# waleedbinkhalid74/cnn-gp

Measured on AMD Instinct MI355X. Metric: kernel entries/s (N×M pairs) + full-Kxx build+solve wall-clock, MNIST 28×28, higher is better.
Workload: dtype f64; 1 GPU; mnist_paper_convnet_gp Kxx 4096x4096, tiles 1024; n=4096, tile=1024, parallelism=tiles-dp1

## Files before the change

### cnn-gp_amd/csrc/net_walk.inc

```
    for (long long u = advance(); u < end; u = advance()) {
        if (tid == 0) grab = atomicAdd(ctr, 1ull);
        Pairs pr;
        pr.tab = pair_tab;
        pr.u0 = u;
        pr.red = red_part;
        if constexpr (NP == 2) {
            const int q = __builtin_amdgcn_readfirstlane(tid >> 7);
            unsigned iq = 0, jq = 0;
            bool vq = false, wq = false, any = false;
#pragma unroll
            for (int s = 0; s < UN; ++s) {
                unsigned is = 0, js = 0;
                const bool vs = u + s < end && unit_pair(p, u + s, is, js);
                const bool ws = vs && !(p.same && js <= is);
                any |= ws;
                if (s == q) {
                    iq = is;
                    jq = js;
                    vq = vs;
                    wq = ws;
                }
            }
            if (!any) {
                if (p.final_stage && p.same && (tid & (kNT - 1)) == 0 && vq && jq == iq)
                    p.out[(long long)iq * p.ldo + iq] = p.kdiag[iq];
                continue;
            }
            Pairs ph;
            ph.tab = pair_tab;
            ph.u0 = u + q;
            ph.red = red_part + q * (kNT / 64);
            ph.i = __builtin_amdgcn_readfirstlane(vq ? iq : 0u);
            ph.j = __builtin_amdgcn_readfirstlane(vq ? jq : 0u);
            T* lh = lds + q * p.lds_elems;
            const int ht = tid & (kNT - 1);
            if constexpr (PID < 0) {
                for (int k = 0; k < p.nops; ++k) {
                    const cgp_net_op op = load_op(ops_c(p.ops) + k);
                    net_op<T, EX, DU, 1>(lh, op, p, ph, ht);
                    lds_barrier();
                }
            } else {
                prog_ops<T, DU, 1, PID, 0, CGP_WALK_LEAN>(lh, p, ph, ht, prog_recs, hx);
            }
            if (p.final_stage && ht == 0 && vq) {
                if (wq) {
                    const T v = lh[p.final_slot];
                    p.out[(long long)ph.i * p.ldo + ph.j] = v;
                    if (p.same) p.out[(long long)ph.j * p.ldo + ph.i] = v;
                } else if (ph.j == ph.i) {
                    p.out[(long long)ph.i * p.ldo + ph.i] = p.kdiag[ph.i];
                }
            }
        } else {
            if constexpr (NP == 1) {
                if (!unit_pair(p, u, pr.i, pr.j)) continue;
                pr.i = __builtin_amdgcn_readfirstlane(pr.i);
                pr.j = __builtin_amdgcn_readfirstlane(pr.j);
                if (p.same && pr.j <= pr.i) {
                    if (p.final_stage && pr.j == pr.i && tid == 0)
                        p.out[(long long)pr.i * p.ldo + pr.i] = p.kdiag[pr.i];
                    continue;
                }
            } else {
                if (tid < NP) {
                    unsigned iq = 0, jq = 0;
                    unit_pair(p, u + tid, iq, jq);
                    pair_tab[tid] = iq < p.n1 ? iq : p.n1 - 1;
                    pair_tab[kMaxNP + tid] = jq < p.n2 ? jq : p.n2 - 1;
                }
                pr.i = pr.j = 0;
                lds_barrier();
            }
            if constexpr (PID < 0) {
                for (int k = 0; k < p.nops; ++k) {
                    const cgp_net_op op = load_op(ops_c(p.ops) + k);
                    net_op<T, EX, DU, NP>(lds, op, p, pr, tid);
                    lds_barrier();
                }
            } else {
                prog_ops<T, DU, NP, PID, 0, CGP_WALK_LEAN>(lds, p, pr, tid, prog_recs, hx);
            }
            if (p.final_stage) {
                if constexpr (NP == 1) {
                    if (tid == 0) {
                        const T v = lds[p.final_slot];
                        p.out[(long long)pr.i * p.ldo + pr.j] = v;
                        if (p.same) p.out[(long long)pr.j * p.ldo + pr.i] = v;
                    }
                } else if (tid < NP) {
                    unsigned iq, jq;
                    if (u + tid < end && unit_pair(p, u + tid, iq, jq)) {
                        if (!p.same || jq > iq) {
                            const T v = lds[tid * p.lds_elems + p.final_slot];
                            p.out[(long long)iq * p.ldo + jq] = v;
                            if (p.same) p.out[(long long)jq * p.ldo + iq] = v;
                        } else if (jq == iq) {
                            p.out[(long long)iq * p.ldo + iq] = p.kdiag[iq];
                        }
                    }
                }
            }
        }
        lds_barrier();
    }
```

### cnn-gp_amd/csrc/netfuse.hip

```cpp

#include "cgp_common.h"


#include <map>
#include <mutex>
#include <utility>
#include <algorithm>
#include <climits>

using namespace cgp;

namespace {

constexpr int kNT = 128;
constexpr int kSplit = 2;
template <int NP>
constexpr int kNTof = NP == 2 ? kSplit * kNT : kNT;
template <int NP>
constexpr int kUnitsOf = NP == 2 ? kSplit : NP;
constexpr int kSTL = 3;
constexpr int kST = 1 << kSTL;
constexpr int kEw = 4;

constexpr int pick_r(int lines, int len, int taps, int s, int epi, int nt) {
// ... 1046 lines not shown

#define CGP_NET_RES_CASE(h, w)                                                        \
    case res_index(h, w):                                                             \
        if constexpr (CGP_NET_FITS(h, w)) net_elem<T, EX, DU, KIND, h, w, NP>(lds, op, p, pr); \
        break;

template <typename T, bool EX, bool DU, int KIND, int NP>
__device__ __forceinline__ void net_elem_dispatch(T* __restrict__ lds, const cgp_net_op& op,
                                                  const NetP<T>& p, const Pairs& pr) {
    if constexpr (KIND == CGP_NET_RELU || (KIND == CGP_NET_LINEAR && NP > 1)) {
        switch (op.code) {
            CGP_NET_RESOLUTIONS(CGP_NET_RES_CASE)
        default:
            if constexpr (NP == 1) net_elem<T, EX, DU, KIND, 0, 0, 1>(lds, op, p, pr);
            break;
        }
    } else if constexpr (NP == 1) {
        net_elem<T, EX, DU, KIND, 0, 0, 1>(lds, op, p, pr);
    }
}

template <typename T, bool EX, bool DU, int NP>
__device__ __forceinline__ void net_op(T* __restrict__ lds, const cgp_net_op& op,
                                       const NetP<T>& p, const Pairs& pr, int tid) {
    if (op.zero_halo) {
#pragma unroll
        for (int q = 0; q < NP; ++q) {
            const int qa = NP == 1 ? 0 : q * p.lds_elems;
            zero_halos<T, kNT>(lds + qa, op.dst, op.zero_halo & 0xffff, op.h, op.w,
                                     op.ws_out, tid);
            zero_halos<T, kNT>(lds + qa, op.dst2, (unsigned)op.zero_halo >> 16, op.h, op.w,
                       op.ws_out, tid);
        }
    }
    switch (op.kind) {
    case CGP_NET_CONV:
        switch (op.code & CGP_NET_CODE_GEOMETRY) {
            CGP_NET_GEOMETRIES(CGP_NET_CASE)
        default:
            break;
        }
        break;
    case CGP_NET_RELU:
        net_elem_dispatch<T, EX, DU, CGP_NET_RELU, NP>(lds, op, p, pr);
        break;
    case CGP_NET_MOMENTS:
        net_elem_dispatch<T, EX, DU, CGP_NET_MOMENTS, NP>(lds, op, p, pr);
        break;
    case CGP_NET_LINEAR:
        net_elem_dispatch<T, EX, DU, CGP_NET_LINEAR, NP>(lds, op, p, pr);
        break;
    case CGP_NET_LOAD:
        net_move<T, CGP_NET_LOAD, NP>(lds, op, p, pr);
        break;
    case CGP_NET_STORE:
        net_move<T, CGP_NET_STORE, NP>(lds, op, p, pr);
        break;
    default:
        break;
    }
}

#ifndef CGP_NET_PRESCALE
#define CGP_NET_PRESCALE 1
#endif
constexpr bool kNetPrescale = CGP_NET_PRESCALE != 0;
struct ProgOp {
    int kind, code, src, dst, add, ws_in, ws_out, relu, h, w, dst2, zero_halo;
};
struct ProgInfo {
    int first, nops, pairs, dual, lds_elems, sizes;
};
#include "net_programs.h"
constexpr int kNumProgs = sizeof(kProgs) / sizeof(kProgs[0]);

struct ProgRec {
    double weight, bias;
    const void* var_x;
    const void* var_y;
    const void* var2_x;
    const void* var2_y;
};
template <int PID>
constexpr int kRecsOf = PID >= 0 ? kProgs[PID < 0 ? 0 : PID].nops : 1;

template <int PID, int K>
__device__ __forceinline__ cgp_net_op prog_op(const ProgRec* recs) {
    constexpr ProgOp o = kProgOps[kProgs[PID].first + K];
    const ProgRec& rt = recs[K];
    cgp_net_op op;
    op.kind = o.kind;
    op.code = o.code;
    op.src = o.src;
    op.dst = o.dst;
    op.add = o.add;
    op.ws_in = o.ws_in;
    op.ws_out = o.ws_out;
    op.relu = o.relu;
    op.h = o.h;
    op.w = o.w;
    op.div_m = 0;
    op.div_s = 0;
    op.dst2 = o.dst2;
    op.zero_halo = o.zero_halo;
    op.weight = rt.weight;
    op.bias = rt.bias;
    op.var_x = rt.var_x;
    op.var_y = rt.var_y;
    op.var2_x = rt.var2_x;
    op.var2_y = rt.var2_y;
    return op;
}
template <int PID, int K, int NP>
struct ProgGeo {
    static constexpr ProgOp o = kProgOps[kProgs[PID].first + K];
    static constexpr GeoRow g = kGeoTable[o.code & CGP_NET_CODE_GEOMETRY];
    using G = NG<g.h, g.w, g.ho, g.wo, g.taps, g.s, g.off, NP>;
};
__host__ __device__ inline bool lean_rec_ok(double w, double b) {
    return w >= 0.0 && w <= 0x1p60 && b >= 0x1p-60 && b <= 0x1p60;
}
constexpr int kMaxProgOps = 24;
struct LeanOp {
    bool nocap = false, half = false, dbl = false;
};
struct ProgLean {
    LeanOp op[kMaxProgOps] = {};
    unsigned dbl_mask = 0;
    int capfree = 0, addfree = 0;
    int nend = 0, end_lo[4] = {}, end_hi[4] = {};
    bool bad = false;
};
struct LeanFact {
    int lo = 0, hi = 0;
    bool nonneg = false, halved = false;
};
constexpr bool lean_overlap(int lo, int hi, int lo2, int hi2) { return lo < hi2 && lo2 < hi; }
constexpr bool op_is_sum(const ProgOp& o) {
    return o.kind == CGP_NET_CONV && (o.code & CGP_NET_CODE_SUM) != 0;
}
constexpr int op_src_hi(const ProgOp& o) {
    if (o.kind == CGP_NET_CONV) return o.src + kGeoTable[o.code & CGP_NET_CODE_GEOMETRY].h * o.ws_in;
    if (o.kind == CGP_NET_RELU || o.kind == CGP_NET_LINEAR || o.kind == CGP_NET_STORE)
        return o.src + o.h * o.ws_in;
    return o.src;
}
constexpr bool op_reads_add(const ProgOp& o) {
    return (o.kind == CGP_NET_CONV || o.kind == CGP_NET_RELU) ? o.add >= 0
                                                              : o.kind == CGP_NET_LINEAR;
}
constexpr bool op_writes_dst(const ProgOp& o) { return o.kind != CGP_NET_STORE; }
constexpr int op_ext(const ProgOp& o) { return o.h * o.ws_out; }
constexpr bool lean_can_halve(const ProgOp* ops, int n, int k, int lo, int hi, bool* end) {
    *end = false;
    for (int m = k + 1; m < n; ++m) {
        const ProgOp& r = ops[m];
        if (op_reads_add(r) && lean_overlap(lo, hi, r.add, r.add + op_ext(r))) return false;
        if (lean_overlap(lo, hi, r.src, op_src_hi(r)) &&
            !(r.kind == CGP_NET_CONV && r.src == lo && op_src_hi(r) <= hi))
            return false;
        if (op_is_sum(r)) continue;
        if (op_writes_dst(r) && lean_overlap(lo, hi, r.dst, r.dst + op_ext(r))) {
            if (r.dst <= lo && r.dst + op_ext(r) >= hi) return true;
            return false;
        }
        if (r.dst2 >= 0 && lean_overlap(lo, hi, r.dst2, r.dst2 + op_ext(r))) {
            if (r.dst2 <= lo && r.dst2 + op_ext(r) >= hi) return true;
            return false;
        }
    }
    if (op_is_sum(ops[k]))
        return k + 1 < n && ops[k + 1].kind == CGP_NET_CONV &&
               (ops[k + 1].code & CGP_NET_CODE_FROM_SUM) != 0 && ops[k + 1].src == lo;
    *end = true;
    return true;
}
constexpr ProgLean prog_lean(int pid) {
    ProgLean L{};
    const ProgInfo I = kProgs[pid];
    const ProgOp* ops = kProgOps + I.first;
    if (I.nops > kMaxProgOps) {
        L.bad = true;
        return L;
    }
    if (I.pairs > 2 || I.dual) return L;
    constexpr int kMaxFacts = 8;
    LeanFact f[kMaxFacts] = {};
    int nf = 0;
    auto find = [&](int lo, int hi) -> const LeanFact* {
        for (int n = 0; n < nf; ++n)
            if (f[n].lo == lo && hi <= f[n].hi) return &f[n];
        return nullptr;
    };
    auto touches_halved = [&](int lo, int hi) {
        for (int n = 0; n < nf; ++n)
            if (f[n].halved && lean_overlap(lo, hi, f[n].lo, f[n].hi)) return true;
        return false;
    };
    auto write = [&](int lo, int hi, bool nonneg, bool halved) {
        int m = 0;
        for (int n = 0; n < nf; ++n)
            if (!lean_overlap(lo, hi, f[n].lo, f[n].hi)) f[m++] = f[n];
        nf = m;
        if (!nonneg) return;
        if (nf == kMaxFacts) {
            if (halved) L.bad = true;
            return;
        }
        f[nf].lo = lo;
        f[nf].hi = hi;
        f[nf].nonneg = nonneg;
        f[nf].halved = halved;
        ++nf;
    };
    for (int k = 0; k < I.nops; ++k) {
        const ProgOp& o = ops[k];
        const int ext = op_ext(o);
        const LeanFact* fs = find(o.src, op_src_hi(o));
        const LeanFact* fa = op_reads_add(o) ? find(o.add, o.add + ext) : nullptr;
        const bool add_nn = !op_reads_add(o) || (fa && fa->nonneg);
        if (op_reads_add(o) && touches_halved(o.add, o.add + ext)) L.bad = true;
        if (o.kind != CGP_NET_CONV && op_src_hi(o) > o.src && touches_halved(o.src, op_src_hi(o)))
            L.bad = true;
        if (o.kind == CGP_NET_CONV) {
            if (touches_halved(o.src, op_src_hi(o)) && !(fs && fs->halved)) L.bad = true;
            const bool src_nn = fs && fs->nonneg;
            L.op[k].dbl = fs && fs->halved;
            if (L.op[k].dbl) L.dbl_mask |= 1u << k;
            bool half = false;
            if (o.relu) {
                L.op[k].nocap = true;
                ++L.capfree;
                bool end = false;
                half = src_nn && o.add < 0 && o.dst2 < 0 &&
                       lean_can_halve(ops, I.nops, k, o.dst, o.dst + ext, &end);
                if (half && end) {
                    if (L.nend == 4) {
                        half = false;
                    } else {
                        L.end_lo[L.nend] = o.dst;
                        L.end_hi[L.nend++] = o.dst + ext;
                    }
                }
                L.op[k].half = half;
                L.addfree += half;
            }
            write(o.dst, o.dst + ext, (o.relu || src_nn) && add_nn, half);
            if (o.dst2 >= 0) write(o.dst2, o.dst2 + ext, true, false);
        } else if (o.kind == CGP_NET_RELU) {
            write(o.dst, o.dst + ext, add_nn, false);
        } else if (o.kind == CGP_NET_LINEAR) {
            write(o.dst, o.dst + ext, false, false);
            if (o.dst2 >= 0) write(o.dst2, o.dst2 + ext, true, false);
        } else if (o.kind == CGP_NET_MOMENTS || o.kind == CGP_NET_LOAD) {
            write(o.dst, o.dst + ext, false, false);
        }
    }
    return L;
}
template <int PID>
struct LeanOf {
    static constexpr ProgLean L = prog_lean(PID < 0 ? 0 : PID);
    static_assert(!L.bad, "prog_lean: a program the slot walk does not cover");
};
#define CGP_LEAN_ROW(k) LeanOf<k>::L,
constexpr ProgLean kLeanTab[] = {CGP_NET_PROGRAMS(CGP_LEAN_ROW)};
#undef CGP_LEAN_ROW
bool lean_final_clash(int pid, int final_slot) {
    const ProgLean& L = kLeanTab[pid];
    for (int n = 0; n < L.nend; ++n)
        if (final_slot >= L.end_lo[n] && final_slot < L.end_hi[n]) return true;
    return false;
}
template <typename T, int PID>
constexpr bool kLeanProg = PID >= 0 && kReluLean && sizeof(T) == 8 &&
                           LeanOf<PID>::L.capfree + LeanOf<PID>::L.addfree > 0;

constexpr bool op_separable(const ProgOp& o) {
    if (o.kind != CGP_NET_CONV) return false;
    const GeoRow& g = kGeoTable[o.code & CGP_NET_CODE_GEOMETRY];
    const bool point = g.taps == 1 && g.off == 0;
    const bool reduce = g.ho == 1 && g.wo == 1 && g.off == 0 && g.taps == g.h && g.taps == g.w;
    return !point && !reduce && g.taps > 3;
}
constexpr int prog_hoist_op(int pid) {
    const ProgInfo I = kProgs[pid];
    if (I.pairs > 2) return -1;
    int first = -1;
    for (int k = 0; k < I.nops; ++k) {
        const ProgOp& o = kProgOps[I.first + k];
        if (!op_separable(o)) continue;
        if (first < 0) first = k;
        const ProgOp& f = kProgOps[I.first + first];
        if ((o.code & CGP_NET_CODE_GEOMETRY) != (f.code & CGP_NET_CODE_GEOMETRY) ||
            o.ws_in != f.ws_in || o.ws_out != f.ws_out)
            return -1;
    }
    return first;
}
template <typename T, int PID>
constexpr bool kHoistProg = CGP_NET_HOIST != 0 && PID >= 0 && sizeof(T) == 8 &&
                            prog_hoist_op(PID < 0 ? 0 : PID) >= 0;

struct NoGeo {
    enum { HO = 0, WO = 1, R3 = 1, NG3 = 0 };
};
template <int PID, int HK, bool ON>
struct HoistGeo {
    using G = NoGeo;
};
template <int PID, int HK>
struct HoistGeo<PID, HK, true> {
    using G = typename ProgGeo<PID, HK, 1>::G;
};

template <typename T, bool DU, int NP, int PID, int K, bool LEAN = false>
__device__ __forceinline__ void prog_ops(T* __restrict__ lds, const NetP<T>& p, const Pairs& pr,
                                         int tid, const ProgRec* recs,
                                         const ConvHoist<T>& hx) {
    constexpr ProgInfo I = kProgs[PID];
    if constexpr (K < I.nops) {
        constexpr ProgOp o = kProgOps[I.first + K];
        constexpr LeanOp lean = LEAN ? LeanOf<PID>::L.op[K] : LeanOp{};
        const cgp_net_op op = prog_op<PID, K>(recs);
        if constexpr (o.zero_halo != 0) {
#pragma unroll
            for (int q = 0; q < NP; ++q) {
                const int qa = q * I.lds_elems;
                zero_halos<T, kNT>(lds + qa, o.dst, o.zero_halo & 0xffff, o.h, o.w,
                                         o.ws_out, tid);
                zero_halos<T, kNT>(lds + qa, o.dst2, (unsigned)o.zero_halo >> 16, o.h, o.w,
                                         o.ws_out,
                           tid);
            }
        }
        if constexpr (o.kind == CGP_NET_CONV) {
            static_assert(!lean.half || (o.relu && o.add < 0 && o.dst2 < 0), "halved output");
            constexpr bool hoist = kHoistProg<T, PID> && op_separable(o);
            net_conv<T, false, DU, typename ProgGeo<PID, K, NP>::G, kNetPrescale, lean.nocap,
                     lean.half, hoist>(lds, op, p, pr, &hx);
        } else if constexpr (o.kind == CGP_NET_MOMENTS && NP == 1 && CGP_NET_MOMENTS_BATCH != 0 &&
                             o.h * o.w <= CGP_NET_MOMENTS_MAXHW) {
            constexpr int hk = prog_hoist_op(PID);
            using HG = typename HoistGeo<PID, hk, (hk >= 0)>::G;
            constexpr ProgOp hc = kProgOps[I.first + (hk < 0 ? 0 : hk)];
            constexpr bool items = CGP_NET_MOMENTS_ITEMS != 0 && kHoistProg<T, PID> &&
                                   o.ws_out == hc.ws_out && o.h == HG::HO && o.w == HG::WO &&
                                   HG::NG3 * HG::R3 == HG::HO;
            net_moments<T, DU, o.h, o.w, o.ws_out, o.dst, items, HG>(lds, op, p, pr, hx);
        } else if constexpr (o.kind == CGP_NET_RELU || o.kind == CGP_NET_LINEAR ||
                             o.kind == CGP_NET_MOMENTS) {
            net_elem<T, false, DU, o.kind, o.h, o.w, NP>(lds, op, p, pr);
        } else if constexpr (o.kind == CGP_NET_LOAD || o.kind == CGP_NET_STORE) {
            if constexpr (CGP_NET_MOVE_C)
                net_move_c<T, o.kind, NP, o.h, o.w, o.kind == CGP_NET_LOAD ? o.dst : o.src,
                           o.kind == CGP_NET_LOAD ? o.ws_out : o.ws_in>(lds, op, p, pr);
            else
                net_move<T, o.kind, NP>(lds, op, p, pr);
        }
        lds_barrier();
        prog_ops<T, DU, NP, PID, K + 1, LEAN>(lds, p, pr, tid, recs, hx);
    }
}
int prog_match(const cgp_net_op* ops, int nops, int pairs, int dual, int lds_elems,
               int itemsize) {
    for (int k = 0; k < kNumProgs; ++k) {
        const ProgInfo& I = kProgs[k];
        if (I.nops != nops || I.pairs != pairs || I.dual != dual || I.lds_elems != lds_elems ||
            !(I.sizes & itemsize))
            continue;
        bool eq = true;
        for (int n = 0; n < nops && eq; ++n) {
            const ProgOp& o = kProgOps[I.first + n];
            const cgp_net_op& r = ops[n];
            eq = o.kind == r.kind && o.code == r.code && o.src == r.src && o.dst == r.dst &&
                 o.add == r.add && o.ws_in == r.ws_in && o.ws_out == r.ws_out &&
                 o.relu == r.relu && o.h == r.h && o.w == r.w && o.dst2 == r.dst2 &&
                 o.zero_halo == r.zero_halo;
        }
        if (eq) return k + 1;
    }
    return 0;
}

template <typename T, bool EX, bool DU, int WPE, int NP, int PID = -1>
__global__ __launch_bounds__(kNTof<NP>) __attribute__((amdgpu_waves_per_eu(WPE))) void net_kernel(const NetP<T> p) {
    extern __shared__ __align__(16) unsigned char smem_raw[];
    __shared__ unsigned pair_tab[2 * kMaxNP];
    __shared__ T red_part[kUnitsOf<NP> * (kNT / 64)];
    T* lds = reinterpret_cast<T*>(smem_raw);
    const int tid = threadIdx.x;
    constexpr int UN = kUnitsOf<NP>;
    for (int e = tid; e < UN * p.lds_elems; e += kNTof<NP>) lds[e] = T(0);
    if (tid < UN * (kNT / 64)) red_part[tid] = T(0);
    __shared__ ProgRec prog_recs[kRecsOf<PID>];
    __shared__ long long next_u[2];
    __shared__ int lean_flag;
    static_assert(sizeof(pair_tab) + sizeof(red_part) + sizeof(prog_recs) + sizeof(next_u) +
                      sizeof(lean_flag) <= kStaticLds,
                  "static LDS beyond the reserve the host checks count (kStaticLds)");
    if constexpr (PID >= 0) {
        const ProgOp* po = kProgOps + kProgs[PID < 0 ? 0 : PID].first;
        for (int k = tid; k < kRecsOf<PID>; k += kNTof<NP>) {
            const cgp_net_op& r = p.ops[k];
            const ProgOp& o = po[k];
            const double qs =
                kNetPrescale && kQuarter<T, false> && o.kind == CGP_NET_CONV && o.relu ? 0.25 : 1.0;
            double ws = qs;
            if constexpr (kLeanProg<T, PID>) {
                bool ok = true;
                for (int n = 0; n < kRecsOf<PID>; ++n)
                    if (po[n].kind == CGP_NET_CONV)
                        ok = ok && lean_rec_ok(p.ops[n].weight, p.ops[n].bias);
                if (ok && ((LeanOf<PID>::L.dbl_mask >> k) & 1u)) ws *= 2.0;
                if (k == 0) lean_flag = ok;
            }
            prog_recs[k] = ProgRec{r.weight * ws, r.bias * qs, r.var_x, r.var_y, r.var2_x,
                                   r.var2_y};
        }
    }
    lds_barrier();
    const unsigned xcd = blockIdx.x % 8;
    const long long span = p.uend - p.ubeg;
    const long long per = ((span + 7) / 8 + UN - 1) / UN * UN;
    const long long beg = p.ubeg + (long long)xcd * per;
    const long long end = beg + per < p.uend ? beg + per : p.uend;
    int adv = 0;
    unsigned long long* ctr = p.work + xcd;
    unsigned long long grab = 0;
    if (tid == 0) grab = atomicAdd(ctr, 1ull);
    auto advance = [&]() {
        if (tid == 0) next_u[adv] = beg + (long long)grab * UN;
        lds_barrier();
        const long long v = next_u[adv];
        adv ^= 1;
        return v;
    };
    ConvHoist<T> hx{};
    if constexpr (kHoistProg<T, PID>) {
        static_assert(NP <= 2, "hoisted decode: one-pair code");
        constexpr int hk = prog_hoist_op(PID < 0 ? 0 : PID);
        constexpr ProgOp ho = kProgOps[kProgs[PID < 0 ? 0 : PID].first + hk];
        T* lh = lds;
        if constexpr (NP == 2) lh += __builtin_amdgcn_readfirstlane(tid >> 7) * p.lds_elems;
        hx = conv_hoist<T, typename ProgGeo<PID < 0 ? 0 : PID, hk, 1>::G>(lh, p, tid & (kNT - 1),
                                                                        ho.ws_in, ho.ws_out, ho.src,
                                                                        ho.dst);
    }
    if constexpr (kLeanProg<T, PID>) {
        if (__builtin_amdgcn_readfirstlane(lean_flag) != 0) {
#define CGP_WALK_LEAN true
#include "net_walk.inc"
#undef CGP_WALK_LEAN
            return;
        }
    }
#define CGP_WALK_LEAN false
#include "net_walk.inc"
#undef CGP_WALK_LEAN
}

constexpr int net_wpe(long long lds_bytes, int cap = 5, int waves = kNT / 64) {
    const long long wg = (160LL * 1024) / (lds_bytes + kStaticLds);
    const long long w = wg * waves / 4;
    return w < 3 ? 3 : (w > cap ? cap : (int)w);
}
constexpr int kProgWpeMax = 5;

template <typename T, int NP>
const void* net_fn_np(bool du, long long lds_bytes) {
    switch (net_wpe(lds_bytes, 5, kNTof<NP> / 64)) {
    case 3: return du ? (const void*)net_kernel<T, false, true, 3, NP>
                      : (const void*)net_kernel<T, false, false, 3, NP>;
    case 4: return du ? (const void*)net_kernel<T, false, true, 4, NP>
                      : (const void*)net_kernel<T, false, false, 4, NP>;
    default:
        return du ? (const void*)net_kernel<T, false, true, 4, NP>
                  : (const void*)net_kernel<T, false, false, 5, NP>;
    }
}
template <typename T>
const void* net_fn(bool ex, bool du, int np, long long lds_bytes) {
    if (ex) {
        if (np != 1) return nullptr;
        return du ? (const void*)net_kernel<T, true, true, 3, 1>
                  : (const void*)net_kernel<T, true, false, 3, 1>;
    }
    if constexpr (sizeof(T) == 8) {
        switch (np) {
        case 1: return net_fn_np<T, 1>(du, lds_bytes);
        case 2: return net_fn_np<T, 2>(du, lds_bytes);
        case 4: return net_fn_np<T, 4>(du, lds_bytes);
        case 16: return net_fn_np<T, 16>(du, lds_bytes);
        default: return nullptr;
        }
    }
    switch (np) {
    case 1: return du ? (const void*)net_kernel<T, false, true, 4, 1>
                      : (const void*)net_kernel<T, false, false, 5, 1>;
    case 2: return du ? (const void*)net_kernel<T, false, true, 4, 2>
                      : (const void*)net_kernel<T, false, false, 5, 2>;
    case 4: return du ? (const void*)net_kernel<T, false, true, 4, 4>
                      : (const void*)net_kernel<T, false, false, 5, 4>;
    case 16: return du ? (const void*)net_kernel<T, false, true, 4, 16>
                       : (const void*)net_kernel<T, false, false, 5, 16>;
    default: return nullptr;
    }
}

template <typename T, int PID>
const void* prog_fn_one() {
    constexpr ProgInfo I = kProgs[PID];
    if constexpr ((I.sizes & (int)sizeof(T)) == 0) {
        return nullptr;
    } else {
        constexpr long long bytes =
            (long long)I.lds_elems * (long long)sizeof(T) * kUnitsOf<I.pairs>;
        constexpr int wpe = sizeof(T) == 8 ? net_wpe(bytes, kProgWpeMax, kNTof<I.pairs> / 64)
                                           : (I.dual ? 4 : 5);
        return (const void*)net_kernel<T, false, I.dual != 0, wpe, I.pairs, PID>;
    }
}
template <typename T>
const void* prog_fn(int pid) {
    switch (pid) {
#define CGP_PROG_CASE(k) \
    case k: return prog_fn_one<T, k>();
        CGP_NET_PROGRAMS(CGP_PROG_CASE)
#undef CGP_PROG_CASE
    default: return nullptr;
    }
}

int net_threads(int np) { return np == 2 ? kNTof<2> : kNT; }
int net_units(int np) { return np == 2 ? kUnitsOf<2> : np; }

int net_occupancy(const void* fn, int lds_bytes, int threads) {
    if (lds_bytes > 64 * 1024 &&
        hipFuncSetAttribute(fn, hipFuncAttributeMaxDynamicSharedMemorySize, lds_bytes) !=
            hipSuccess) {
        (void)hipGetLastError();
        return 0;
    }
    int n = 0;
    if (hipOccupancyMaxActiveBlocksPerMultiprocessor(&n, fn, threads, lds_bytes) != hipSuccess) {
        (void)hipGetLastError();
        return 0;
    }
    return n;
}

template <typename T>
int net_occupancy_for(int lds_bytes, int flags, int np) {
    const void* fn = net_fn<T>(flags & CGP_FLAG_EXACT_RELU, flags & CGP_FLAG_NET_DUAL, np,
                               (long long)lds_bytes * net_units(np));
    return fn ? net_occupancy(fn, lds_bytes * net_units(np), net_threads(np)) : 0;
}

unsigned long long* work_counters(hipStream_t s) {
    constexpr int kSlots = 64;
    struct Ring {
        unsigned long long* buf = nullptr;
        unsigned next = 0;
    };
    static std::mutex mu;
    static std::map<std::pair<int, hipStream_t>, Ring> rings;
    int dev = 0;
    if (stream_device(s, &dev) != hipSuccess) {
        (void)hipGetLastError();
        return nullptr;
    }
    unsigned long long* slot = nullptr;
    {
        std::lock_guard<std::mutex> lock(mu);
        Ring& r = rings[{dev, s}];
        if (!r.buf) {
            int cur = 0;
            hipError_t e = hipGetDevice(&cur);
            if (e == hipSuccess && cur != dev) e = hipSetDevice(dev);
            if (e == hipSuccess)
                e = hipMalloc(&r.buf, sizeof(unsigned long long) * 8 * kSlots);
            if (cur != dev) (void)hipSetDevice(cur);
            if (e != hipSuccess) {
                (void)hipGetLastError();
                r.buf = nullptr;
                return nullptr;
            }
        }
        slot = r.buf + 8 * (r.next++ % kSlots);
    }
    if (hipMemsetAsync(slot, 0, sizeof(unsigned long long) * 8, s) != hipSuccess) {
        (void)hipGetLastError();
        return nullptr;
    }
    return slot;
}

template <typename T>
int net_launch(const NetP<T>& p, bool ex, bool du, int np, long long lds_bytes, int program,
               void* stream) {
    const long long wg_bytes = lds_bytes * net_units(np);
    const void* fn = program > 0 && !ex ? prog_fn<T>(program - 1) : net_fn<T>(ex, du, np, wg_bytes);
    if (!fn) return fail(CGP_EINVAL, "net: no instantiation for %d pairs per workgroup", np);
    const int per_cu = net_occupancy(fn, (int)wg_bytes, net_threads(np));
    if (per_cu <= 0)
        return fail(CGP_EINVAL, "net: kernel cannot be resident with %lld B LDS", wg_bytes);
    const long long groups = (p.uend - p.ubeg + net_units(np) - 1) / net_units(np);
    long long grid = (long long)per_cu * device_cus();
    if (grid > groups) grid = groups;
    grid = (grid + 7) / 8 * 8;
    NetP<T> arg = p;
    hipStream_t s = as_stream(stream);
    arg.work = work_counters(s);
    if (!arg.work) return fail(CGP_EHIP, "net: work counters");
    void* args[] = {&arg};
    const hipError_t e = hipLaunchKernel(fn, dim3((unsigned)grid), dim3(net_threads(np)), args,
                                         (size_t)wg_bytes, s);
    if (e != hipSuccess) return fail(CGP_EHIP, "net_kernel launch: %s", hipGetErrorString(e));
    return check_launch("net_kernel");
}

template <typename T>
int net_impl(const cgp_net_args* a, void* stream) {
    if (!a) return fail(CGP_EINVAL, "net: args is NULL");
    if (!a->x || !a->y || !a->out || !a->ops || a->nops <= 0)
        return fail(CGP_EINVAL, "net: NULL pointer or empty op list");
    if (a->n1 <= 0 || a->n2 <= 0 || a->n1 >= (1LL << 31) || a->n2 >= (1LL << 31) ||
        a->ldo < a->n2)
        return fail(CGP_EINVAL, "net: bad sizes n1=%lld n2=%lld ldo=%lld", (long long)a->n1,
                    (long long)a->n2, (long long)a->ldo);
    if (a->same && (a->n1 != a->n2 || !a->kdiag))
        return fail(CGP_EINVAL, "net: same tile needs n1 == n2 and kdiag");
    if (a->channels <= 0 || a->h <= 0 || a->w <= 0)
        return fail(CGP_EINVAL, "net: bad image shape");
    const long long lds_bytes = (long long)a->lds_elems * (long long)sizeof(T);
    if (a->lds_elems <= 0 || lds_bytes + kStaticLds > 160 * 1024)
        return fail(CGP_EINVAL, "net: LDS footprint %lld bytes out of range", lds_bytes);
    if (a->final_slot < 0 || a->final_slot >= a->lds_elems || a->hs < 0 ||
        a->hs >= a->lds_elems || a->part < 0 || a->part + 2 > a->lds_elems)
        return fail(CGP_EINVAL, "net: slot offsets out of range");
    NetP<T> p;
    p.x = static_cast<const T*>(a->x);
    p.y = static_cast<const T*>(a->y);
    p.out = static_cast<T*>(a->out);
    p.kdiag = static_cast<const T*>(a->kdiag);
    p.ops = a->ops;
    p.ldo = a->ldo;
    p.n1 = (unsigned)a->n1;
    p.n2 = (unsigned)a->n2;
    p.nbi = (unsigned)((a->n1 + kST - 1) / kST);
    p.nbj = (unsigned)((a->n2 + kST - 1) / kST);
    const long long tiles = a->same ? (long long)p.nbi * (p.nbi + 1) / 2
                                    : (long long)p.nbi * p.nbj;
    if (tiles * kST * kST >= (1LL << 40)) return fail(CGP_EINVAL, "net: tile too large");
    p.units = tiles * kST * kST;
    p.nops = a->nops;
    p.channels = a->channels;
    p.hw_in = a->h * a->w;
    p.same = a->same;
    p.final_slot = a->final_slot;
    p.hs = a->hs;
    p.part = a->part;
    p.lds_elems = a->lds_elems;
    p.exact = (a->flags & CGP_FLAG_EXACT_RELU) ? 1 : 0;
    const int np = a->pairs <= 0 ? 1 : a->pairs;
    if (np != 1 && np != 2 && np != 4 && np != kMaxNP)
        return fail(CGP_EINVAL, "net: %d pairs per workgroup (1, 2, 4 or 16)", np);
    if (lds_bytes * net_units(np) + kStaticLds > 160 * 1024)
        return fail(CGP_EINVAL, "net: %d pairs need %lld B LDS (+ %lld B static)", np,
                    lds_bytes * net_units(np), kStaticLds);
    if (np > 1 && (a->n1 > a->n2 ? a->n1 : a->n2) * (8LL * net_threads(np) / np) *
                          (long long)sizeof(T) >= (1LL << 32))
        return fail(CGP_EINVAL, "net: %lld images too many for %d pairs per workgroup",
                    (long long)(a->n1 > a->n2 ? a->n1 : a->n2), np);
    if (a->unit_begin == 0 && a->unit_end == 0) {
        p.ubeg = 0;
        p.uend = p.units;
    } else {
        p.ubeg = a->unit_begin;
        p.uend = a->unit_end;
    }
    if (p.ubeg < 0 || p.uend > p.units || p.ubeg >= p.uend || p.ubeg % np)
        return fail(CGP_EINVAL, "net: unit range [%lld, %lld) of %lld", (long long)p.ubeg,
                    (long long)p.uend, (long long)p.units);
    p.final_stage = a->final_stage;
    const bool du = (a->flags & CGP_FLAG_NET_DUAL) != 0;
    const int prog = a->program;
    if (prog < 0 || prog > kNumProgs)
        return fail(CGP_EINVAL, "net: program %d of %d", prog, kNumProgs);
    if (prog > 0) {
        const ProgInfo& I = kProgs[prog - 1];
        if (I.nops != a->nops || I.pairs != np || I.dual != (du ? 1 : 0) ||
            I.lds_elems != a->lds_elems || !(I.sizes & (int)sizeof(T)))
            return fail(CGP_EINVAL, "net: program %d does not fit this op list", prog);
        if (kReluLean && sizeof(T) == 8 && !p.exact && a->final_stage &&
            lean_final_clash(prog - 1, a->final_slot))
            return fail(CGP_EINVAL, "net: final slot %d of program %d is a map slot",
                        (int)a->final_slot, prog);
    }
    return net_launch<T>(p, p.exact != 0, du, np, lds_bytes, prog, stream);
}

}

extern "C" {

int cgp_net_geometry(int32_t h, int32_t w, int32_t ho, int32_t wo, int32_t taps,
                     int32_t stride, int32_t offset) {
    for (int k = 0; k < kNumGeo; ++k) {
        const GeoRow& g = kGeoTable[k];
        if (g.h == h && g.w == w && g.ho == ho && g.wo == wo && g.taps == taps &&
            g.s == stride && g.off == offset)
            return k;
    }
    return -1;
}

int cgp_net_resolution(int32_t h, int32_t w) { return res_index(h, w); }

size_t cgp_net_op_size(void) { return sizeof(cgp_net_op); }
size_t cgp_net_args_size(void) { return sizeof(cgp_net_args); }

int cgp_net_supertile(void) { return kST; }
int cgp_net_var_form(void) { return kNetVarForm; }

int cgp_net_units(int32_t pairs) { return net_units(pairs <= 0 ? 1 : pairs); }

int cgp_net_hs_elems(int32_t code) {
    return (code >= 0 && code < kNumGeo) ? kGeoTable[code].hs_elems : -1;
}

int cgp_net_occupancy(int32_t lds_bytes, int32_t f64, int32_t flags, int32_t pairs) {
    if (pairs <= 0) pairs = 1;
    if (lds_bytes <= 0 || (long long)lds_bytes * pairs > 160 * 1024) return 0;
    return f64 ? net_occupancy_for<double>(lds_bytes, flags, pairs)
               : net_occupancy_for<float>(lds_bytes, flags, pairs);
}

int cgp_net_static_lds(void) { return (int)kStaticLds; }

int cgp_net_validate(const cgp_net_op* ops, int32_t nops, int32_t pairs) {
    if (!ops || nops <= 0) return fail(CGP_EINVAL, "net_validate: NULL or empty op list");
    const int np = pairs <= 0 ? 1 : pairs;
    auto geo = [](const cgp_net_op& r) -> const GeoRow* {
        const int g = r.code & CGP_NET_CODE_GEOMETRY;
        return r.kind == CGP_NET_CONV && r.code >= 0 && g < kNumGeo ? &kGeoTable[g] : nullptr;
    };
    for (int k = 0; k < nops; ++k) {
        const cgp_net_op& r = ops[k];
        const bool sum = r.kind == CGP_NET_CONV && r.code >= 0 && (r.code & CGP_NET_CODE_SUM);
        const bool from = r.kind == CGP_NET_CONV && r.code >= 0 && (r.code & CGP_NET_CODE_FROM_SUM);
        if (sum) {
            const GeoRow* g = geo(r);
            const bool point = g && g->taps == 1 && g->off == 0;
            const bool reduce = g && g->ho == 1 && g->wo == 1 && g->off == 0 &&
                                g->taps == g->h && g->taps == g->w;
            if (!g || g->taps <= 3 || point || reduce)
                return fail(CGP_EINVAL, "net_validate: op %d: CGP_NET_CODE_SUM needs a separable "
                                        "conv (more than 3 taps, not pointwise, not a reduction)", k);
            if (r.add >= 0 || r.dst2 >= 0)
                return fail(CGP_EINVAL, "net_validate: op %d: CGP_NET_CODE_SUM with an addend or "
                                        "a second output", k);
            if (np > 2)
                return fail(CGP_EINVAL, "net_validate: op %d: CGP_NET_CODE_SUM in a %d-pair stage "
                                        "(one pair per workgroup or half only)", k, np);
            if (k + 1 >= nops || !(ops[k + 1].kind == CGP_NET_CONV && ops[k + 1].code >= 0 &&
                                   (ops[k + 1].code & CGP_NET_CODE_FROM_SUM)) ||
                ops[k + 1].src != r.dst)
                return fail(CGP_EINVAL, "net_validate: op %d: CGP_NET_CODE_SUM not followed by the "
                                        "CGP_NET_CODE_FROM_SUM reduction of its map", k);
            for (int m = k + 2; m < nops; ++m)
                if (ops[m].src == r.dst || ops[m].add == r.dst)
                    return fail(CGP_EINVAL, "net_validate: op %d reads the map of SUM op %d, "
                                            "which is never stored", m, k);
        }
        if (from) {
            const GeoRow* g = geo(r);
            const bool reduce = g && g->ho == 1 && g->wo == 1 && g->off == 0 &&
                                g->taps == g->h && g->taps == g->w;
            if (!reduce || np > 2)
                return fail(CGP_EINVAL, "net_validate: op %d: CGP_NET_CODE_FROM_SUM needs a "
                                        "one-pair full-map reduction", k);
            if (k == 0 || !(ops[k - 1].kind == CGP_NET_CONV && ops[k - 1].code >= 0 &&
                            (ops[k - 1].code & CGP_NET_CODE_SUM)))
                return fail(CGP_EINVAL, "net_validate: op %d: CGP_NET_CODE_FROM_SUM without a "
                                        "CGP_NET_CODE_SUM conv before it", k);
        }
    }
    return CGP_OK;
}

int cgp_net_program(const cgp_net_op* ops, int32_t nops, int32_t pairs, int32_t flags,
                    int32_t lds_elems, int32_t itemsize) {
    if (!ops || nops <= 0) return 0;
    return prog_match(ops, nops, pairs <= 0 ? 1 : pairs, (flags & CGP_FLAG_NET_DUAL) ? 1 : 0,
                      lds_elems, itemsize);
}

int cgp_net_program_lean(const cgp_net_op* ops, int32_t nops, int32_t pairs, int32_t flags,
                         int32_t lds_elems, int32_t itemsize, int32_t* capfree,
                         int32_t* addfree) {
    if (!kReluLean || !ops || nops <= 0 || itemsize != 8 || (flags & CGP_FLAG_EXACT_RELU))
        return 0;
    const int k = prog_match(ops, nops, pairs <= 0 ? 1 : pairs,
                             (flags & CGP_FLAG_NET_DUAL) ? 1 : 0, lds_elems, itemsize);
    if (k <= 0) return 0;
    for (int n = 0; n < nops; ++n)
        if (ops[n].kind == CGP_NET_CONV && !lean_rec_ok(ops[n].weight, ops[n].bias)) return 0;
    const ProgLean& L = kLeanTab[k - 1];
    if (capfree) *capfree = L.capfree;
    if (addfree) *addfree = L.addfree;
    return 1;
}

int cgp_net_f64(const cgp_net_args* args, void* stream) { return net_impl<double>(args, stream); }
int cgp_net_f32(const cgp_net_args* args, void* stream) { return net_impl<float>(args, stream); }

}
```

Before: 129.4 million pairs/s.

## Fold final reduce-conv into tail value and compute unit pair once per group

For hoisted f64 programs whose last op is a full-window reduce conv from a sum, the final op is skipped. The output is computed directly from the per-wave partial sums as weight*sum+bias, which drops that op's LDS pass and the trailing loop barrier. For the two-pair split path, the pair indices are decoded once per group of two units and the second is derived by incrementing j, avoiding a second unit_pair decode. It adds a host check that the final slot matches the last op's output. Removing the barrier relies on the partial-sum buffer not being overwritten before it is read.

```diff
diff --git a/cnn-gp_amd/csrc/net_walk.inc b/cnn-gp_amd/csrc/net_walk.inc
--- a/cnn-gp_amd/csrc/net_walk.inc
+++ b/cnn-gp_amd/csrc/net_walk.inc
@@ -8,17 +8,36 @@
             const int q = __builtin_amdgcn_readfirstlane(tid >> 7);
             unsigned iq = 0, jq = 0;
             bool vq = false, wq = false, any = false;
+            if constexpr (kUnitOnce<T, PID, NP>) {
+                static_assert(UN == 2, "kUnitOnce: groups of two units");
+                unsigned i0 = 0, j0 = 0;
+                unit_pair(p, u, i0, j0);
 #pragma unroll
-            for (int s = 0; s < UN; ++s) {
-                unsigned is = 0, js = 0;
-                const bool vs = u + s < end && unit_pair(p, u + s, is, js);
-                const bool ws = vs && !(p.same && js <= is);
-                any |= ws;
-                if (s == q) {
-                    iq = is;
-                    jq = js;
-                    vq = vs;
-                    wq = ws;
+                for (int s = 0; s < UN; ++s) {
+                    unsigned is = 0, js = 0;
+                    const bool vs = u + s < end && unit_next(p, u + s, i0, j0 + s, is, js);
+                    const bool ws = vs && !(p.same && js <= is);
+                    any |= ws;
+                    if (s == q) {
+                        iq = is;
+                        jq = js;
+                        vq = vs;
+                        wq = ws;
+                    }
+                }
+            } else {
+#pragma unroll
+                for (int s = 0; s < UN; ++s) {
+                    unsigned is = 0, js = 0;
+                    const bool vs = u + s < end && unit_pair(p, u + s, is, js);
+                    const bool ws = vs && !(p.same && js <= is);
+                    any |= ws;
+                    if (s == q) {
+                        iq = is;
+                        jq = js;
+                        vq = vs;
+                        wq = ws;
+                    }
                 }
             }
             if (!any) {
@@ -45,7 +64,11 @@
             }
             if (p.final_stage && ht == 0 && vq) {
                 if (wq) {
-                    const T v = lh[p.final_slot];
+                    T v;
+                    if constexpr (kTailProg<T, PID>)
+                        v = prog_tail_value<T, PID>(prog_recs, ph.red);
+                    else
+                        v = lh[p.final_slot];
                     p.out[(long long)ph.i * p.ldo + ph.j] = v;
                     if (p.same) p.out[(long long)ph.j * p.ldo + ph.i] = v;
                 } else if (ph.j == ph.i) {
@@ -84,7 +107,11 @@
             if (p.final_stage) {
                 if constexpr (NP == 1) {
                     if (tid == 0) {
-                        const T v = lds[p.final_slot];
+                        T v;
+                        if constexpr (kTailProg<T, PID>)
+                            v = prog_tail_value<T, PID>(prog_recs, pr.red);
+                        else
+                            v = lds[p.final_slot];
                         p.out[(long long)pr.i * p.ldo + pr.j] = v;
                         if (p.same) p.out[(long long)pr.j * p.ldo + pr.i] = v;
                     }
@@ -102,5 +129,5 @@
                 }
             }
         }
-        lds_barrier();
+        if constexpr (!kTailProg<T, PID>) lds_barrier();
     }
diff --git a/cnn-gp_amd/csrc/netfuse.hip b/cnn-gp_amd/csrc/netfuse.hip
--- a/cnn-gp_amd/csrc/netfuse.hip
+++ b/cnn-gp_amd/csrc/netfuse.hip
@@ -1372,6 +1372,51 @@
 constexpr bool kHoistProg = CGP_NET_HOIST != 0 && PID >= 0 && sizeof(T) == 8 &&
                             prog_hoist_op(PID < 0 ? 0 : PID) >= 0;
 
+#ifndef CGP_NET_TAIL
+#define CGP_NET_TAIL 1
+#endif
+constexpr bool prog_tail_ok(int pid) {
+    const ProgInfo I = kProgs[pid];
+    if (I.pairs > 2 || I.dual || I.nops < 2) return false;
+    const ProgOp& o = kProgOps[I.first + I.nops - 1];
+    if (o.kind != CGP_NET_CONV || !(o.code & CGP_NET_CODE_FROM_SUM)) return false;
+    const GeoRow& g = kGeoTable[o.code & CGP_NET_CODE_GEOMETRY];
+    const bool reduce = g.ho == 1 && g.wo == 1 && g.off == 0 && g.taps == g.h && g.taps == g.w;
+    return reduce && !o.relu && o.add < 0 && o.dst2 < 0 && o.zero_halo == 0 &&
+           op_is_sum(kProgOps[I.first + I.nops - 2]);
+}
+template <typename T, int PID>
+constexpr bool kTailProg = CGP_NET_TAIL != 0 && kHoistProg<T, PID> &&
+                           prog_tail_ok(PID < 0 ? 0 : PID);
+int prog_tail_slot(int pid, int itemsize) {
+    if (CGP_NET_TAIL == 0 || CGP_NET_HOIST == 0 || itemsize != 8) return -1;
+    if (prog_hoist_op(pid) < 0 || !prog_tail_ok(pid)) return -1;
+    return kProgOps[kProgs[pid].first + kProgs[pid].nops - 1].dst;
+}
+template <typename T, int PID>
+__device__ __forceinline__ T prog_tail_value(const ProgRec* recs, const void* red) {
+    constexpr int K = kProgs[PID].nops - 1;
+    const T* part = static_cast<const T*>(red);
+    T tot = part[0];
+#pragma unroll
+    for (int k = 1; k < kNT / 64; ++k) tot += part[k];
+    return fma_t(T(recs[K].weight), tot, T(recs[K].bias));
+}
+
+#ifndef CGP_NET_UNIT_ONCE
+#define CGP_NET_UNIT_ONCE 1
+#endif
+template <typename T, int PID, int NP>
+constexpr bool kUnitOnce = CGP_NET_UNIT_ONCE != 0 && kHoistProg<T, PID> && NP == 2;
+template <typename T>
+__device__ __forceinline__ bool unit_next(const NetP<T>& p, long long u, unsigned iu,
+                                          unsigned ju, unsigned& i, unsigned& j) {
+    i = iu;
+    j = ju;
+    return u < p.units && i < p.n1 && j < p.n2;
+}
+static_assert(kST % 2 == 0, "kUnitOnce: an even unit and its successor share a supertile row");
+
 struct NoGeo {
     enum { HO = 0, WO = 1, R3 = 1, NG3 = 0 };
 };
@@ -1389,7 +1434,7 @@
                                          int tid, const ProgRec* recs,
                                          const ConvHoist<T>& hx) {
     constexpr ProgInfo I = kProgs[PID];
-    if constexpr (K < I.nops) {
+    if constexpr (K < I.nops - (kTailProg<T, PID> ? 1 : 0)) {
         constexpr ProgOp o = kProgOps[I.first + K];
         constexpr LeanOp lean = LEAN ? LeanOf<PID>::L.op[K] : LeanOp{};
         const cgp_net_op op = prog_op<PID, K>(recs);
@@ -1767,6 +1812,10 @@
             lean_final_clash(prog - 1, a->final_slot))
             return fail(CGP_EINVAL, "net: final slot %d of program %d is a map slot",
                         (int)a->final_slot, prog);
+        const int tail = prog_tail_slot(prog - 1, (int)sizeof(T));
+        if (tail >= 0 && !p.exact && a->final_stage && a->final_slot != tail)
+            return fail(CGP_EINVAL, "net: final slot %d of program %d is not its last op's "
+                                    "output (%d)", (int)a->final_slot, prog, tail);
     }
     return net_launch<T>(p, p.exact != 0, du, np, lds_bytes, prog, stream);
 }
```

Result: no change. 130.0 million pairs/s (median of 6 runs) (+0.5%).
